# sahaRatul/sela

Hardware: NVIDIA H100
Metric: encode+decode MSamples/s (higher is better)
Workload: dtype f64+int64

## Files before the change

### sela_b200/csrc/c_abi.cu

```cuda
#include <algorithm>
#include <atomic>
#include <cmath>
#include <cstdarg>
#include <cstddef>
#include <cstdio>
#include <cstdlib>
#include <cstring>
#include <mutex>
#include <thread>
#include <vector>

#include "lossless.cuh"
#include "pairing.cuh"
#include "search.cuh"
#include "search_guided.cuh"
#include "search_pairing.cuh"
#include "verify.cuh"
#include "window.cuh"

using namespace selab200;

namespace {

thread_local char g_error[512] = "";
// ... 728 lines not shown
            wp.mask = o.windows;
            wp.n = n_windows;
            wp.su = reinterpret_cast<SearchUnit *>(ws + l.window_search);
            wp.key = reinterpret_cast<unsigned long long *>(ws + l.window_keys);
            wp.n_window = o.d_n_window;
            wp.pred = o.d_window_pred;
            wp.trace = o.d_search_trace;
            const bool trace = o.d_search_trace != nullptr;
            if (int rc = stereo ? launch_windows<true>(p, wp, su, n_frames, n_units, o.d_base_words, stream, trace)
                                : launch_windows<false>(p, wp, su, n_frames, n_units, o.d_base_words, stream, trace))
                return rc;
        }
    } else {
        const int rc_units = stereo ? (o.d_trace ? launch_encode_units<true, true>(p, n_units, o.d_trace, stream)
                                                 : launch_encode_units<true, false>(p, n_units, nullptr, stream))
                                    : (o.d_trace ? launch_encode_units<false, true>(p, n_units, o.d_trace, stream)
                                                 : launch_encode_units<false, false>(p, n_units, nullptr, stream));
        if (rc_units)
            return rc_units;
    }
    const unsigned scan_ctas = (unsigned)((n_sub + kScanTile - 1) / kScanTile);
    k_encode_sizes<<<scan_ctas, kScanTile, 0, stream>>>(p);
    if (int rc = launch_check("k_encode_sizes"))
        return rc;
    if (o.before_scan)
        CUDA_TRY(cudaStreamWaitEvent(stream, o.before_scan, 0));
    k_encode_scan<<<scan_ctas, kScanTile, 0, stream>>>(p);
    if (int rc = launch_check("k_encode_scan"))
        return rc;
    CUDA_TRY(cudaMemcpyAsync(d_used, p.residues, 8, cudaMemcpyDeviceToDevice, stream));
    if (pairing) {
        k_pairing_patch<<<(unsigned)((n_sub + 255) / 256), 256, 0, stream>>>(p, q);
        if (int rc = launch_check("k_pairing_patch"))
            return rc;
    }
    if (o.h_fill_after)
        CUDA_TRY(cudaMemcpyAsync(o.h_fill_after, d_used, 8, cudaMemcpyDeviceToHost, stream));
    if (o.after_scan)
        CUDA_TRY(cudaEventRecord(o.after_scan, stream));
    if (o.d_container) {
        k_encode_gather_container<<<(unsigned)((n_sub + 7) / 8), 256, 0, stream>>>(p, o.d_container, o.sub_base);
        return launch_check("k_encode_gather_container");
    }
    k_encode_gather<<<(unsigned)((n_sub + 7) / 8), 256, 0, stream>>>(p);
    return launch_check("k_encode_gather");
}

int launch_rice_decode(const DecodeParams &p, int which, cudaStream_t stream)
{
    const size_t n_sub = (size_t)p.n_frames * p.channels;
    const unsigned blocks = (unsigned)((n_sub + 32 * kRiceWarps - 1) / (32 * kRiceWarps));
    k_rice_decode<kRiceRing, kRiceBatch><<<blocks, 32 * kRiceWarps, 0, stream>>>(p, which);
    return launch_check(which ? "k_rice_decode(res)" : "k_rice_decode(refl)");
}

int rice_split_log2(size_t n_sub)
{
    if (const char *env = std::getenv("SELAB200_RICE_SPLIT")) {
        const long v = std::atol(env);
        if (v <= 0)
            return -1;
        int l = 0;
        while ((1 << (l + 1)) <= v && l < 4)
            l++;
        return l;
    }
    const size_t sms = (size_t)g.sms;
    if (n_sub >= 81 * sms)
        return 0;
    int l = 0;
    while (l < 4 && (n_sub << l) < 270 * sms)
        l++;
    return l;
}

template <int LOG2S>
int launch_split_index(const RiceVsParams &q, size_t n_sub, cudaStream_t stream)
{
    const unsigned blocks = (unsigned)(((n_sub << LOG2S) + 32 * kVsWarps - 1) / (32 * kVsWarps));
    if (int rc = set_smem(k_rice_split_index<LOG2S>, kSplitSmemBytes))
        return rc;
    k_rice_split_index<LOG2S><<<blocks, 32 * kVsWarps, kSplitSmemBytes, stream>>>(q);
    return launch_check("k_rice_split_index");
}

int launch_rice_residues(const DecodeParams &p, void *aux, cudaStream_t stream)
{
    const size_t n_sub = (size_t)p.n_frames * p.channels;
    const int log2s = rice_split_log2(n_sub);
    if (log2s < 0 || (reinterpret_cast<uintptr_t>(p.ws_res) & 15) != 0) {
        CUDA_TRY(cudaMemsetAsync(static_cast<uint32_t *>(aux) + n_sub * 15, 0, n_sub * 4, stream));
        return launch_rice_decode(p, 1, stream);
    }
    RiceVsParams q;
    q.descs = p.descs;
    q.n_sub = (uint32_t)n_sub;
    q.channels = p.channels;
    q.words = p.words;
    q.n_words = p.n_words;
    q.out = p.ws_res;
    q.table = static_cast<uint32_t *>(aux);
    q.flags = q.table + n_sub * 15;
    q.status = p.status;
    int rc = 0;
    switch (log2s) {
    case 0: CUDA_TRY(cudaMemsetAsync(q.flags, 0, n_sub * 4, stream)); break;
    case 1: rc = launch_split_index<1>(q, n_sub, stream); break;
    case 2: rc = launch_split_index<2>(q, n_sub, stream); break;
    case 3: rc = launch_split_index<3>(q, n_sub, stream); break;
    default: rc = launch_split_index<4>(q, n_sub, stream); break;
    }
    if (rc)
        return rc;
    const size_t n_vs = n_sub << log2s;
    const unsigned vs_blocks = (unsigned)((n_vs + 32 * kVsWarps - 1) / (32 * kVsWarps));
    if (int rc2 = set_smem(k_rice_decode_vc, kVcSmemBytes))
        return rc2;
    k_rice_decode_vc<<<vs_blocks, 32 * kVsWarps, kVcSmemBytes, stream>>>(q, log2s);
    if (int rc2 = launch_check("k_rice_decode_vc"))
        return rc2;
    DecodeParams pf = p;
    pf.rice_flags = q.flags;
    return launch_rice_decode(pf, 1, stream);
}

int decode_device(const selab200_subframe_desc *d_descs, uint32_t n_frames, uint32_t channels,
                  const uint32_t *d_words, size_t n_words, int16_t *d_pcm, int32_t *d_status, void *d_ws,
                  size_t ws_bytes, cudaStream_t stream, bool fresh = true)
{
    if (int rc = check_channels(channels))
        return rc;
    if (ws_bytes < selab200_decode_workspace_bytes(n_frames, channels))
        return fail(SELAB200_ERR_ARGUMENT, "decode workspace too small");
    if (fresh)
        CUDA_TRY(cudaMemsetAsync(d_status, 0, sizeof(int32_t), stream));
    if (n_frames == 0)
        return 0;
    const size_t n_sub = (size_t)n_frames * channels;
    DecodeParams p;
    p.descs = d_descs;
    p.n_frames = n_frames;
    p.channels = channels;
    p.words = d_words;
    p.n_words = n_words;
    p.pcm_out = d_pcm;
    p.status = d_status;
    p.ws_q = static_cast<int32_t *>(d_ws);
    p.ws_res = reinterpret_cast<int32_t *>(static_cast<char *>(d_ws) + align256(n_sub * 128 * 4));
    p.seg_index = reinterpret_cast<uint32_t *>(reinterpret_cast<char *>(p.ws_res) + align256(n_sub * kFrame * 4));
    p.rice_flags = nullptr;
    const size_t n_warps = synthesis_warps(n_sub);
    void *rice_aux = reinterpret_cast<char *>(p.seg_index) + align256(n_warps * 32 * 4);
    CUDA_TRY(cudaMemsetAsync(p.seg_index, 0xff, n_warps * 32 * 4, stream));
    const unsigned plan_ctas = (unsigned)((n_sub + kScanTile - 1) / kScanTile);
    k_decode_width_counts<<<plan_ctas, kScanTile, 0, stream>>>(p, static_cast<WidthCounts *>(rice_aux));
    if (int rc = launch_check("k_decode_width_counts"))
        return rc;
    k_decode_plan<<<plan_ctas, kScanTile, 0, stream>>>(p, static_cast<const WidthCounts *>(rice_aux));
    if (int rc = launch_check("k_decode_plan"))
        return rc;
    if (int rc = launch_rice_decode(p, 0, stream))
        return rc;
    if (int rc = launch_rice_residues(p, rice_aux, stream))
        return rc;
    k_synthesise_segments<<<(unsigned)n_warps, 32, 0, stream>>>(p);
    if (int rc = launch_check("k_synthesise_segments"))
        return rc;
    if (channels == 1)
        return 0;
    k_diff_fixup<<<n_frames, 128, 0, stream>>>(p);
    return launch_check("k_diff_fixup");
}

int read_status(cudaStream_t stream, const int32_t *d_status)
{
    CUDA_TRY(cudaMemcpyAsync(&g.h_small->status, d_status, sizeof(int32_t), cudaMemcpyDeviceToHost, stream));
    CUDA_TRY(cudaStreamSynchronize(stream));
    if (g.h_small->status != 0)
        return fail(g.h_small->status, "%s", status_text(g.h_small->status));
    return 0;
}

int verify_device(const selab200_subframe_desc *d_descs, uint32_t n_frames, uint32_t channels, const uint32_t *d_words,
                  size_t n_words, const int16_t *d_ref, selab200_verify_entry *d_entries, unsigned long long *d_count,
                  int32_t *d_status, void *d_ws, size_t ws_bytes, cudaStream_t stream, bool fresh = true,
                  uint32_t frame_base = 0)
{
    if (int rc = check_channels(channels))
        return rc;
    if (ws_bytes < selab200_verify_workspace_bytes(n_frames, channels))
        return fail(SELAB200_ERR_ARGUMENT, "verify workspace too small");
    if ((reinterpret_cast<uintptr_t>(d_ref) & 15) != 0)
        return fail(SELAB200_ERR_ARGUMENT, "source PCM must be 16-byte aligned on the device");
    const size_t n_sub = (size_t)n_frames * channels;
    if (fresh) {
        CUDA_TRY(cudaMemsetAsync(d_status, 0, sizeof(int32_t), stream));
        CUDA_TRY(cudaMemsetAsync(d_count, 0, sizeof(unsigned long long), stream));
        if (n_sub)
            CUDA_TRY(cudaMemsetAsync(d_entries, 0, n_sub * sizeof(selab200_verify_entry), stream));
    }
    if (n_frames == 0)
        return 0;
    const size_t dec_bytes = align256(selab200_decode_workspace_bytes(n_frames, channels));
    int16_t *d_decoded = reinterpret_cast<int16_t *>(static_cast<char *>(d_ws) + dec_bytes);
    if (int rc = decode_device(d_descs, n_frames, channels, d_words, n_words, d_decoded, d_status, d_ws, dec_bytes,
                               stream, false))
        return rc;
    k_verify_compare<<<n_frames, kVerifyThreads, 0, stream>>>(d_decoded, d_ref, channels, frame_base, d_status,
                                                              d_entries, d_count);
    return launch_check("k_verify_compare");
}

struct VerifyArea {
    unsigned long long *count = nullptr;
    int32_t *status = nullptr;
    selab200_verify_entry *entries = nullptr;
    selab200_subframe_desc *descs = nullptr;
    uint32_t *arena = nullptr;
};

int verify_area(size_t n_sub, size_t arena_words, cudaStream_t stream, VerifyArea &v)
{
    const size_t e_bytes = align256(n_sub * sizeof(selab200_verify_entry));
    const size_t d_bytes = arena_words ? align256(n_sub * sizeof(selab200_subframe_desc)) : 0;
    if (int rc = g.verify.ensure(256 + e_bytes + d_bytes + (arena_words ? arena_words * 4 + 64 : 0)))
        return rc;
    char *b = static_cast<char *>(g.verify.ptr);
    v.count = reinterpret_cast<unsigned long long *>(b);
    v.status = reinterpret_cast<int32_t *>(b + 8);
    v.entries = reinterpret_cast<selab200_verify_entry *>(b + 256);
    v.descs = arena_words ? reinterpret_cast<selab200_subframe_desc *>(b + 256 + e_bytes) : nullptr;
    v.arena = arena_words ? reinterpret_cast<uint32_t *>(b + 256 + e_bytes + d_bytes) : nullptr;
    CUDA_TRY(cudaMemsetAsync(b, 0, 256 + n_sub * sizeof(selab200_verify_entry), stream));
    return 0;
}

bool record_set(const selab200_verify_entry &e) { return e.n_differing != 0; }
bool record_set(const selab200_lossless_entry &e) { return e.words != 0; }

template <typename T>
int collect_records(const unsigned long long *d_count, const int32_t *d_status, const T *d_records, size_t n,
                    cudaStream_t stream, std::vector<T> &out)
{
    out.clear();
    CUDA_TRY(cudaMemcpyAsync(&g.h_small->n_records, d_count, d_status ? 16 : 8, cudaMemcpyDeviceToHost, stream));
    CUDA_TRY(cudaStreamSynchronize(stream));
    const unsigned long long count = g.h_small->n_records;
    const int32_t st = d_status ? g.h_small->records_status : 0;
    if (st != 0)
        return fail(st, "%s", status_text(st));
    if (count == 0)
        return 0;
    std::vector<T> all(n);
    CUDA_TRY(cudaMemcpyAsync(all.data(), d_records, n * sizeof(T), cudaMemcpyDeviceToHost, stream));
    CUDA_TRY(cudaStreamSynchronize(stream));
    out.reserve((size_t)count);
    for (const T &e : all)
        if (record_set(e))
            out.push_back(e);
    return 0;
}

template <typename T>
int deliver_records(const std::vector<T> &records, T *entries, size_t capacity, size_t *n_entries)
{
    *n_entries = records.size();
    if (capacity && !records.empty())
        memcpy(entries, records.data(), std::min(capacity, records.size()) * sizeof(T));
    return 0;
}

}

extern "C" {

int selab200_abi_version(void) { return SELAB200_ABI_VERSION; }
const char *selab200_last_error(void) { return g_error; }
uint64_t selab200_launch_count(void) { return g_launches.load(); }

static int init_slot(int device, int slot)
{
    CUDA_TRY(cudaSetDevice(device));
    cudaDeviceProp prop;
    CUDA_TRY(cudaGetDeviceProperties(&prop, device));
    if (prop.major != 9 || prop.minor != 0)
        return fail(SELAB200_ERR_NO_DEVICE, "device %d is sm_%d%d; this build targets sm_90a only", device,
                    prop.major, prop.minor);
    CUDA_TRY(cudaStreamCreateWithFlags(&g.stream, cudaStreamNonBlocking));
    CUDA_TRY(cudaStreamCreateWithFlags(&g.s_h2d, cudaStreamNonBlocking));
    CUDA_TRY(cudaStreamCreateWithFlags(&g.s_d2h, cudaStreamNonBlocking));
    for (int i = 0; i < kLanes; i++)
        CUDA_TRY(cudaStreamCreateWithFlags(&g.s_compute[i], cudaStreamNonBlocking));
    for (int i = 0; i < kMaxChunks; i++) {
        CUDA_TRY(cudaEventCreateWithFlags(&g.ev_h2d[i], cudaEventDisableTiming));
        CUDA_TRY(cudaEventCreateWithFlags(&g.ev_done[i], cudaEventDisableTiming));
        CUDA_TRY(cudaEventCreateWithFlags(&g.ev_scan[i], cudaEventDisableTiming));
    }
    CUDA_TRY(cudaEventCreateWithFlags(&g.ev_reset, cudaEventDisableTiming));
    g.events = true;
    CUDA_TRY(cudaMallocHost(reinterpret_cast<void **>(&g.h_small), sizeof(Counters)));
    CUDA_TRY(cudaMallocHost(reinterpret_cast<void **>(&g.h_totals), (kMaxChunks + 1) * 8));
    if (int rc = g.small.ensure(256))
        return rc;
    CUDA_TRY(cudaMemcpyToSymbol(d_analysis_windows, analysis_window_table(), sizeof(d_analysis_windows)));
    CUDA_TRY(cudaDeviceSynchronize());
    void *table = nullptr;
    CUDA_TRY(cudaGetSymbolAddress(&table, d_analysis_windows));
    g.windows = static_cast<const double *>(table);
    g.spare = &g_spare_store[slot];
    g.device = device;
    g.sms = prop.multiProcessorCount;
    g.ready = true;
    return 0;
}

static void shutdown_slot()
{
    if (g.device >= 0)
// ... 2095 lines not shown
```

### sela_b200/csrc/kernels.cuh

```cuda
#pragma once

#include "lpc.cuh"
#include "rice.cuh"
#include "rice_vs.cuh"

namespace selab200 {

enum { kMeanPcm = 0, kMeanStereo = 1, kMeanPlanar = 2 };
constexpr int kMeanTile = 64;
constexpr int kMeanSlots = 16;

struct MeanTiling {
    uint32_t units_per_row;
    uint32_t step;
    uint32_t row_stride;
    uint32_t rows_max;
    uint32_t row_words;
};

__host__ __device__ inline MeanTiling mean_tiling(int kind, uint32_t channels)
{
    MeanTiling t;
    uint32_t span = 1;
    if (kind == kMeanPcm) {
// ... 618 lines not shown
    }
    if (lane < (int)(4 - s))
        out[D + lane] = (uint8_t)(src[0] >> (8 * lane));
    else if (lane >= 4 && lane < (int)(4 + s))
        out[D - s + 4ull * n + (lane - 4)] = (uint8_t)(src[n - 1] >> (8 * (4 - s + (lane - 4))));
}

__device__ __forceinline__ void get_words_at_byte(const uint8_t *in, unsigned long long D, uint32_t *dst, uint32_t n)
{
    const int lane = lane_id();
    const uint32_t s = (uint32_t)(D & 3);
    const uint32_t *src = reinterpret_cast<const uint32_t *>(in + (D - s));
    for (uint32_t t0 = lane; t0 < n; t0 += 128) {
        uint32_t v[4];
#pragma unroll
        for (int j = 0; j < 4; j++) {
            const uint32_t t = t0 + 32 * j;
            v[j] = t < n ? (s ? __funnelshift_r(src[t], src[t + 1], 8 * s) : src[t]) : 0u;
        }
#pragma unroll
        for (int j = 0; j < 4; j++)
            if (t0 + 32 * j < n)
                dst[t0 + 32 * j] = v[j];
    }
}

__global__ void __launch_bounds__(256) k_encode_gather_container(EncodeParams p, uint8_t *container,
                                                                 unsigned long long sub_base)
{
    const uint32_t sub = blockIdx.x * 8 + warp_id();
    const uint32_t n_sub = p.n_frames * p.channels;
    if (sub >= n_sub || *reinterpret_cast<volatile int32_t *>(p.status) != 0)
        return;
    const int lane = lane_id();
    const Emit e = choose_unit(p.units, p.channels, sub);
    const selab200_subframe_desc d = p.descs[sub];
    const uint32_t *slot = p.slots + (size_t)e.unit * kSlotWords;
    const unsigned long long g = sub_base + sub;
    const unsigned long long at = container_subframe_byte(g, p.channels, d.refl_offset);
    if (g % p.channels == 0 && lane >= 12 && lane < 16) {
        const uint32_t sync = 0xAA55FF00u;
        container[at - 4 + (lane - 12)] = (uint8_t)(sync >> (8 * (lane - 12)));
    }
    const unsigned long long at2 = at + 7 + 4ull * d.refl_words;
    if (lane < 12) {
        uint8_t v;
        switch (lane) {
        case 0: v = d.channel; break;
        case 1: v = d.subframe_type; break;
        case 2: v = d.parent_channel; break;
        case 3: v = d.refl_rice_param; break;
        case 4: v = (uint8_t)d.refl_words; break;
        case 5: v = (uint8_t)(d.refl_words >> 8); break;
        case 6: v = d.lpc_order; break;
        case 7: v = d.res_rice_param; break;
        case 8: v = (uint8_t)d.res_words; break;
        case 9: v = (uint8_t)(d.res_words >> 8); break;
        case 10: v = (uint8_t)d.samples; break;
        default: v = (uint8_t)(d.samples >> 8); break;
        }
        container[lane < 7 ? at + lane : at2 + (lane - 7)] = v;
    }
    put_words_at_byte(container, at + 7, slot, d.refl_words);
    put_words_at_byte(container, at2 + 5, slot + kSlotReflWords, d.res_words);
}

__global__ void __launch_bounds__(256) k_container_unpack(const uint8_t *container, const selab200_subframe_desc *descs,
                                                          uint32_t n_sub, uint32_t channels, unsigned long long sub_base,
                                                          uint32_t *arena)
{
    const uint32_t sub = blockIdx.x * 8 + warp_id();
    if (sub >= n_sub)
        return;
    const selab200_subframe_desc d = descs[sub];
    const unsigned long long at = container_subframe_byte(sub_base + sub, channels, d.refl_offset);
    get_words_at_byte(container, at + 7, arena + d.refl_offset, d.refl_words);
    get_words_at_byte(container, at + 7 + 4ull * d.refl_words + 5, arena + d.res_offset, d.res_words);
}


__device__ __forceinline__ bool frame_check(const selab200_subframe_desc *fd, uint32_t ch, unsigned long long n_words)
{
    bool ok = true;
    unsigned seen = 0, type_mask = 0;
    for (uint32_t i = 0; i < ch; i++) {
        const selab200_subframe_desc d = fd[i];
        const bool good = desc_ok(d, ch, n_words) && !((seen >> d.channel) & 1);
        ok &= good;
        if (good) {
            seen |= 1u << d.channel;
            type_mask |= (unsigned)(d.subframe_type & 1) << d.channel;
        }
    }
    for (uint32_t i = 0; i < ch && ok; i++) {
        const selab200_subframe_desc d = fd[i];
        if (d.subframe_type == 1 && ((type_mask >> d.parent_channel) & 1))
            ok = false;
    }
    return ok;
}

struct DecodeParams {
    const selab200_subframe_desc *descs;
    uint32_t n_frames, channels;
    const uint32_t *words;
    unsigned long long n_words;
    int16_t *pcm_out;
    int32_t *status;
    int32_t *ws_q;
    int32_t *ws_res;
    uint32_t *seg_index;
    const uint32_t *rice_flags;
};

constexpr int kRiceWarps = 2;
constexpr int kRiceRing = 64, kRiceBatch = 8;
template <int RING, int BATCH>
__global__ void __launch_bounds__(32 * kRiceWarps) k_rice_decode(DecodeParams p, int which)
{
    __shared__ uint32_t ring[kRiceWarps][(RING + 1) * 32];
    const uint32_t sub = blockIdx.x * blockDim.x + threadIdx.x;
    const uint32_t n_sub = p.n_frames * p.channels;
    RiceLaneStream st;
    st.src = p.words;
    st.n_words = 0;
    st.k = 0;
    st.count = 0;
    st.out = nullptr;
    if (sub < n_sub) {
        const selab200_subframe_desc d = p.descs[sub];
        if (!desc_ok(d, p.channels, p.n_words)) {
            raise_status(p.status, SELAB200_ERR_BITSTREAM);
        } else if (which == 0) {
            st.src = p.words + d.refl_offset;
            st.n_words = d.refl_words;
            st.k = d.refl_rice_param;
            st.count = d.lpc_order;
            st.out = p.ws_q + (size_t)sub * 128;
        } else if (!p.rice_flags || p.rice_flags[sub]) {
            st.src = p.words + d.res_offset;
            st.n_words = d.res_words;
            st.k = d.res_rice_param;
            st.count = d.samples;
            st.out = p.ws_res + (size_t)sub * kFrame;
        }
    }
    if (which == 1 && p.rice_flags && __ballot_sync(kFull, st.count != 0) == 0)
        return;
    if (!warp_rice_decode32<RING, BATCH>(ring[warp_id()], st))
        raise_status(p.status, SELAB200_ERR_BITSTREAM);
}

constexpr uint32_t kNoSegment = 0xffffffffu;
constexpr int kMaxTemplates = 2 * kMaxWidth;

struct WidthCounts {
    uint32_t n[16];
};
struct SegTemplate {
    uint32_t repeats, first_warp;
    uint8_t copies[16], lane0[16];
};

__device__ __forceinline__ int subframe_width(const DecodeParams &p, uint32_t u)
{
    const int order = p.descs[u].lpc_order;
    return segment_width(order > kMaxOrder ? 0 : order);
}

__device__ __forceinline__ uint32_t warp_width_counts(int w, uint32_t (*cnt)[16])
{
    const int lane = lane_id();
    uint32_t rank = 0;
#pragma unroll
    for (int v = 0; v < 16; v++) {
        const unsigned b = __ballot_sync(kFull, w == v);
        if (w == v)
            rank = __popc(b & ((1u << lane) - 1u));
        if (lane == 0)
            cnt[warp_id()][v] = __popc(b);
    }
    return rank;
}

__global__ void __launch_bounds__(kScanTile) k_decode_width_counts(DecodeParams p, WidthCounts *tmp)
{
    __shared__ uint32_t cnt[32][16];
    const uint32_t u = blockIdx.x * kScanTile + threadIdx.x;
    warp_width_counts(u < p.n_frames * p.channels ? subframe_width(p, u) : 0, cnt);
    __syncthreads();
    if (threadIdx.x < 16) {
        uint32_t s = 0;
        for (int w = 0; w < 32; w++)
            s += cnt[w][threadIdx.x];
        tmp[blockIdx.x].n[threadIdx.x] = s;
    }
}

__device__ int segment_templates(uint32_t (&c)[16], SegTemplate *tpl)
{
    int nt = 0;
    uint32_t warp = 0;
    for (;;) {
        SegTemplate t;
        int room = 32;
        uint32_t rep = 0xffffffffu;
#pragma unroll
        for (int v = 15; v >= 1; v--) {
            const uint32_t k = v > kMaxWidth ? 0u : min(c[v], (uint32_t)(room / v));
            t.copies[v] = (uint8_t)k;
            t.lane0[v] = (uint8_t)(32 - room);
            room -= (int)k * v;
            if (k)
                rep = min(rep, c[v] / k);
        }
        if (room == 32)
            return nt;
#pragma unroll
        for (int v = 1; v < 16; v++)
            c[v] -= rep * t.copies[v];
        t.copies[0] = t.lane0[0] = 0;
        t.repeats = rep;
        t.first_warp = warp;
        warp += rep;
        tpl[nt++] = t;
    }
}

__global__ void __launch_bounds__(kScanTile) k_decode_plan(DecodeParams p, const WidthCounts *tmp)
{
    __shared__ uint32_t cnt[32][16];
    __shared__ uint32_t part_all[kScanTile / 16][16], part_before[kScanTile / 16][16];
    __shared__ uint32_t total[16], before[16];
    __shared__ SegTemplate tpl[kMaxTemplates];
    const uint32_t n_units = p.n_frames * p.channels;
    const uint32_t u = blockIdx.x * kScanTile + threadIdx.x;
    const int w = u < n_units ? subframe_width(p, u) : 0;
    const uint32_t rank = warp_width_counts(w, cnt);
    {
        const int v = threadIdx.x & 15, g = threadIdx.x >> 4;
        uint32_t all = 0, pre = 0;
        for (uint32_t b = g; b < gridDim.x; b += kScanTile / 16) {
            const uint32_t x = tmp[b].n[v];
            all += x;
            if (b < blockIdx.x)
                pre += x;
        }
        part_all[g][v] = all;
        part_before[g][v] = pre;
    }
    __syncthreads();
    if (threadIdx.x < 16) {
        const int v = threadIdx.x;
        uint32_t all = 0, pre = 0, run = 0;
        for (int g = 0; g < kScanTile / 16; g++)
            all += part_all[g][v], pre += part_before[g][v];
        total[v] = all;
        before[v] = pre;
        for (int x = 0; x < 32; x++) {
            const uint32_t c = cnt[x][v];
            cnt[x][v] = run;
            run += c;
        }
    }
    __syncthreads();
    if (threadIdx.x == 0) {
        uint32_t c[16];
#pragma unroll
        for (int v = 0; v < 16; v++)
            c[v] = v ? total[v] : 0u;
        segment_templates(c, tpl);
    }
    __syncthreads();
    if (u >= n_units)
        return;
    const uint32_t r = before[w] + cnt[warp_id()][w] + rank;
    uint32_t acc = 0;
    int t = 0;
    for (;; t++) {
        const uint32_t m = tpl[t].repeats * tpl[t].copies[w];
        if (r < acc + m)
            break;
        acc += m;
    }
    const uint32_t k = tpl[t].copies[w], j = r - acc, rep = j / k;
    const uint32_t lane = tpl[t].lane0[w] + (j - rep * k) * (uint32_t)w;
    p.seg_index[((size_t)tpl[t].first_warp + rep) * 32 + lane] = u;
}

__host__ __device__ inline size_t synthesis_warps(size_t n_sub) { return n_sub / 2 + 1; }

__global__ void __launch_bounds__(32) k_synthesise_segments(DecodeParams p)
{
    __shared__ __align__(16) SegSmem sm;
    const uint32_t ch = p.channels;
    const int lane = lane_id();
    const uint32_t entry = p.seg_index[(size_t)blockIdx.x * 32 + lane];
    const unsigned starts = __ballot_sync(kFull, entry != kNoSegment);
    if (!(starts & 1u))
        return;
    const int start = 31 - __clz(starts & (0xffffffffu >> (31 - lane)));
    const uint32_t sub = __shfl_sync(kFull, entry, start);
    const int seg = __popc(starts & ((1u << start) - 1u));
    const int n_seg = __popc(starts);
    const int k = lane - start;
    const uint32_t frame = sub / ch, pos = sub % ch;
    const selab200_subframe_desc *fd = p.descs + (size_t)frame * ch;
    const int n = subframe_width(p, sub);
    const bool exists = k < n;

    const bool frame_ok = frame_check(fd, ch, p.n_words);
    if (!frame_ok && k == 0)
        raise_status(p.status, SELAB200_ERR_BITSTREAM);
    const selab200_subframe_desc mine = fd[pos];
    const bool proc = exists && frame_ok;
    const bool diff = proc && mine.subframe_type == 1;
    int16_t *out = p.pcm_out + (size_t)frame * kFrame * ch;
    int32_t *row = p.ws_res + (size_t)sub * kFrame;
    if (k == 0) {
        sm.row_res[seg] = row;
        sm.row_out[seg] = diff ? static_cast<void *>(row) : static_cast<void *>(out + mine.channel);
        sm.row_mode[seg] = !proc ? 0 : diff ? 2 : 1;
    }
    __syncwarp();
    segment_synthesis(sm, start, k, n, seg, n_seg, proc ? mine.lpc_order : 0, p.ws_q + (size_t)sub * 128, ch);

    if (exists && !frame_ok) {
        for (int t = k; t < kFrame; t += n)
            out[(size_t)t * ch + pos] = 0;
    }
}

__global__ void __launch_bounds__(128) k_diff_fixup(DecodeParams p)
{
    const uint32_t frame = blockIdx.x, ch = p.channels;
    const selab200_subframe_desc *fd = p.descs + (size_t)frame * ch;
    bool any = false;
    for (uint32_t pos = 0; pos < ch; pos++)
        any |= fd[pos].subframe_type == 1;
    if (!any || !frame_check(fd, ch, p.n_words))
        return;
    int16_t *out = p.pcm_out + (size_t)frame * kFrame * ch;
    for (uint32_t pos = 0; pos < ch; pos++) {
        const selab200_subframe_desc d = fd[pos];
        if (d.subframe_type != 1)
            continue;
        const int32_t *diff = p.ws_res + ((size_t)frame * ch + pos) * kFrame;
        for (int t = threadIdx.x; t < kFrame; t += blockDim.x)
            out[(size_t)t * ch + d.channel] =
                (int16_t)(uint16_t)((uint32_t)out[(size_t)t * ch + d.parent_channel] - (uint32_t)diff[t]);
    }
}


struct Row17 {
    __align__(16) int16_t a[kHistoryPad + kFrame];
    uint32_t lo[(kHistoryPad + kFrame) / 32];
    __device__ __forceinline__ Signal stage(const int32_t *src)
    {
        const int lane = lane_id();
        for (int i = lane; i < kHistoryPad / 2; i += 32)
            reinterpret_cast<uint32_t *>(a)[i] = 0;
        if (lane < kHistoryPad / 32)
            lo[lane] = 0;
        stage_17bit_row(src, a + kHistoryPad, lo + kHistoryPad / 32);
        __syncwarp();
        return Signal{a + kHistoryPad, lo + kHistoryPad / 32};
    }
};

__global__ void __launch_bounds__(32) k_lpc_residues(const int32_t *samples, const double *means, uint32_t n_sub,
                                                     uint8_t *order_out, int32_t *q_out, int32_t *residues)
{
    __shared__ __align__(16) AnalysisScratch scratch;
    __shared__ __align__(16) CoefSmem cf;
    __shared__ __align__(16) Row17 row;
    const uint32_t sub = blockIdx.x;
    const int lane = lane_id();
    const Signal sig = row.stage(samples + (size_t)sub * kFrame);
    warp_autocorrelation(sig, scratch, means[sub]);
    warp_schur(scratch);
    const int order = warp_order_and_quantise(scratch, cf);
    warp_coefficients(cf, scratch.t(), order);
    warp_fir_residual<true>(sig, cf, order, reinterpret_cast<uint32_t *>(scratch.ring), residues + (size_t)sub * kFrame);
    for (int i = lane; i < kMaxOrder; i += 32)
        q_out[(size_t)sub * kMaxOrder + i] = i < order ? cf.q[i] : 0;
    if (lane == 0)
        order_out[sub] = (uint8_t)order;
}

template <bool CHECK = false>
__global__ void __launch_bounds__(32) k_fir_probe(const int32_t *samples, const int32_t *orders, const long long *c,
                                                  int wide, int32_t *residues, uint8_t *ties)
{
    __shared__ __align__(16) AnalysisScratch scratch;
    __shared__ __align__(16) CoefSmem cf;
    __shared__ __align__(16) Row17 row;
    const uint32_t sub = blockIdx.x;
    const int lane = lane_id();
    const int32_t *src = samples + (size_t)sub * kFrame;
    Signal sig = row.stage(src);
    if (!wide) {
        for (int j = lane; j < kFrame; j += 32)
            row.a[kHistoryPad + j] = (int16_t)src[j];
        sig.lo = nullptr;
    }
    const int order = orders[sub];
    for (int i = lane; i < 112; i += 32) {
        const long long v = i < order ? c[(size_t)sub * (kMaxOrder + 1) + i + 1] : 0;
        cf.clo[i] = (uint32_t)v;
        cf.chi[i] = (int32_t)(v >> 32);
    }
    __syncwarp();
    uint32_t *planes = reinterpret_cast<uint32_t *>(scratch.ring);
    int32_t *res = residues + (size_t)sub * kFrame;
    const bool tie = wide ? warp_fir_residual<true, CHECK>(sig, cf, order, planes, res)
                          : warp_fir_residual<false, CHECK>(sig, cf, order, planes, res);
    if (CHECK && lane == 0)
        ties[sub] = tie;
}

__global__ void __launch_bounds__(32) k_lpc_samples(const int32_t *residues, uint32_t n_sub, const uint8_t *order_in,
                                                    const int32_t *q_in, int32_t *samples)
{
    __shared__ __align__(16) SegSmem sm;
    const uint32_t sub = blockIdx.x;
    const int lane = lane_id();
    const int order = min((int)order_in[sub], kMaxOrder);
    const int n = segment_width(order);
    if (lane == 0) {
        sm.row_res[0] = residues + (size_t)sub * kFrame;
        sm.row_out[0] = samples + (size_t)sub * kFrame;
        sm.row_mode[0] = 2;
    }
    __syncwarp();
    segment_synthesis(sm, 0, lane, n, 0, 1, lane < n ? order : 0, q_in + (size_t)sub * kMaxOrder, 1);
}

__global__ void k_quantise_probe(const double *k, uint32_t n, int32_t *out)
{
    const uint32_t i = blockIdx.x * blockDim.x + threadIdx.x;
    if (i >= n)
        return;
    const double kv = k[i];
    out[4 * (size_t)i + 0] = quantise_reflection(0, kv);
    out[4 * (size_t)i + 1] = quantise_reflection(1, kv);
    out[4 * (size_t)i + 2] = quantise_reflection(2, kv);
    out[4 * (size_t)i + 3] = reflection_significant(kv) ? 1 : 0;
}

__global__ void k_selftest_scaling(uint32_t *mismatches)
{
    const int s = (int)(blockIdx.x * blockDim.x + threadIdx.x) - 65535;
    if (s > 65535)
        return;
    if (__double_as_longlong(sample_to_x(s)) != __double_as_longlong(sample_to_x_div(s)))
        atomicAdd(mismatches, 1u);
}

__global__ void __launch_bounds__(32) k_rice_encode(const int32_t *values, const uint32_t *counts, uint32_t pitch,
                                                    uint32_t *k_out, uint32_t *n_words_out, uint32_t *words,
                                                    uint32_t words_stride, int32_t *status)
{
    const uint32_t st = blockIdx.x;
    const int32_t *v = values + (size_t)st * pitch;
    const int n = (int)counts[st];
    RiceChoice c = warp_rice_choose(v, n);
    if (lane_id() == 0) {
        k_out[st] = c.k;
        n_words_out[st] = c.words;
    }
    if (c.words > words_stride) {
        if (lane_id() == 0)
            raise_status(status, SELAB200_ERR_CAPACITY);
        return;
    }
    warp_rice_pack(v, n, c, words + (size_t)st * words_stride);
}

__global__ void __launch_bounds__(32 * kRiceWarps) k_rice_decode_streams(
    const uint32_t *words, const uint32_t *n_words, uint32_t words_stride, const uint32_t *k,
    const uint32_t *counts, uint32_t n_streams, int32_t *out, uint32_t out_stride, int32_t *status)
{
    __shared__ uint32_t ring[kRiceWarps][(kRiceRing + 1) * 32];
    const uint32_t st_i = blockIdx.x * blockDim.x + threadIdx.x;
    RiceLaneStream st;
    st.src = words;
    st.n_words = 0;
    st.k = 0;
    st.count = 0;
    st.out = nullptr;
    if (st_i < n_streams) {
        if (k[st_i] >= 32 || counts[st_i] > out_stride || n_words[st_i] > words_stride) {
            raise_status(status, SELAB200_ERR_BITSTREAM);
        } else {
            st.src = words + (size_t)st_i * words_stride;
            st.n_words = n_words[st_i];
            st.k = k[st_i];
            st.count = counts[st_i];
            st.out = out + (size_t)st_i * out_stride;
        }
    }
    warp_rice_decode32<kRiceRing, kRiceBatch>(ring[warp_id()], st);
}

}
```

### sela_b200/csrc/lpc.cuh

```cuda
#pragma once

#include "common.cuh"
#include "lpc_tables.cuh"

namespace selab200 {

struct CoefSmem {
    uint32_t clo[112];
    int32_t  chi[112];
    int32_t  q[104];
};
struct AnalysisScratch {
    double ring[256];
    double ac[128];
    __device__ __forceinline__ double *kk() { return ring; }
    __device__ __forceinline__ double *t() { return ring + 104; }
};
using LpcSmem = AnalysisScratch;
constexpr size_t kCoefAlias = 208 * sizeof(double);

__device__ __forceinline__ long long coef_at(const CoefSmem &cf, int j)
{
    return (long long)(((unsigned long long)(uint32_t)cf.chi[j - 1] << 32) | cf.clo[j - 1]);
}
// ... 369 lines not shown
                    sum = mad_wide_s32(T[k][r], 1 << (8 * k), sum);
                const uint32_t top = (uint32_t)T[4][r] + ((uint32_t)T[5][r] << 8) + ((uint32_t)T[6][r] << 16) +
                                     ((uint32_t)T[7][r] << 24);
                sum += (unsigned long long)top << 32;
                out[e] = s[e] - (int32_t)((long long)sum >> kQ);
                if constexpr (CHECK)
                    tie |= (int32_t)((long long)sum >> kQ) + (int32_t)((long long)((1ull << kQ) - sum) >> kQ) != 0;
            }
            *reinterpret_cast<int2 *>(res + i) = make_int2(out[0], out[1]);
        }
    }
    __syncwarp();
    if constexpr (CHECK)
        return __any_sync(kFull, tie);
    return false;
}

constexpr int kTapsPerLane = 8;
constexpr int kMaxWidth = (kMaxOrder + kTapsPerLane - 1) / kTapsPerLane;
constexpr int kSegBlock = 16;
constexpr int kSegRow = 20;
static_assert(kSegBlock % kTapsPerLane == 0, "the register of slot 0 must be static inside a block");

__device__ __forceinline__ int segment_width(int order)
{
    return order <= kTapsPerLane ? 1 : (order + kTapsPerLane - 1) / kTapsPerLane;
}

struct SegSmem {
    int32_t q[32 * kTapsPerLane];
    union {
        double t[32 * kTapsPerLane];
        int32_t out[32 * kSegRow];
    };
    int32_t in[2][32 * kSegRow];
    const int32_t *row_res[32];
    void *row_out[32];
    int row_mode[32];
};

__device__ __forceinline__ void segment_coefficients(SegSmem &sm, int start, int k, int n, int order, int order_max,
                                                     uint32_t (&cl)[kTapsPerLane], uint32_t (&ch)[kTapsPerLane])
{
    double *t = sm.t + kTapsPerLane * start;
    const int32_t *q = sm.q + kTapsPerLane * start;
    const bool live = order > 1 && k < n;
    for (int i = 0; i < order_max; i++) {
        if (live && i < order) {
            const double ki = dequantise(i, q[i]);
            const int half = i >> 1;
            for (int j = k; j < half; j += n) {
                double a = t[j];
                double b = t[i - 1 - j];
                t[j] = dadd(a, dmul(ki, b));
                t[i - 1 - j] = dadd(b, dmul(ki, a));
            }
            if (k == 0) {
                if (i & 1) {
                    double mid = t[half];
                    t[half] = dadd(mid, dmul(mid, ki));
                }
                t[i] = ki;
            }
        }
        __syncwarp();
    }
    const double scale = 34359738368.0;
#pragma unroll
    for (int m = 0; m < kTapsPerLane; m++) {
        const int j = kTapsPerLane * k + m;
        const long long v = (live && j < order) ? __double2ll_rz(dmul(scale, -t[j])) : 0;
        cl[m] = (uint32_t)v;
        ch[m] = (uint32_t)((unsigned long long)v >> 32);
    }
    __syncwarp();
}

struct SegState {
    uint32_t cl[kTapsPerLane];
    uint32_t ch[kTapsPerLane];
    unsigned long long acc[kTapsPerLane];
    uint32_t sp;
    unsigned long long fresh;
};

__device__ __forceinline__ void segment_state(SegState &st, int k, int n, int src)
{
    unsigned long long tot = 0, loc[kTapsPerLane];
#pragma unroll
    for (int m = kTapsPerLane - 1; m >= 0; m--) {
        loc[m] = tot;
        tot += ((unsigned long long)st.ch[m] << 32) | st.cl[m];
    }
    unsigned long long incl = tot;
#pragma unroll
    for (int o = 1; o < 32; o <<= 1) {
        const unsigned long long x = __shfl_down_sync(kFull, incl, o);
        if (k + o < n)
            incl += x;
    }
    const unsigned long long above = incl - tot;
    st.fresh = ~((1ull << (kQ - 1)) + (__shfl_sync(kFull, incl, src) << 31));
#pragma unroll
    for (int m = 0; m < kTapsPerLane; m++)
        st.acc[m] = ((above + loc[m]) << 31) + st.fresh;
}

__device__ __forceinline__ unsigned long long segment_tap(unsigned long long acc, uint32_t cl, uint32_t ch, uint32_t sp)
{
    unsigned long long d;
    asm("{\n\t.reg .u32 lo, hi;\n\t"
        "mov.b64 {lo, hi}, %4;\n\t"
        "mad.lo.u32 hi, %2, %3, hi;\n\t"
        "mad.lo.cc.u32 lo, %1, %3, lo;\n\t"
        "madc.hi.u32 hi, %1, %3, hi;\n\t"
        "mov.b64 %0, {lo, hi};\n\t}"
        : "=l"(d) : "r"(cl), "r"(ch), "r"(sp), "l"(acc));
    return d;
}

template <bool FIRST>
__device__ __forceinline__ void segment_block(SegState &st, const int32_t *in_row, int32_t *out_row, int src, bool top,
                                              bool first)
{
#pragma unroll
    for (int g = 0; g < kSegBlock; g += 4) {
        const int4 r4 = *reinterpret_cast<const int4 *>(in_row + g);
        const uint32_t r[4] = {(uint32_t)r4.x, (uint32_t)r4.y, (uint32_t)r4.z, (uint32_t)r4.w};
        uint32_t s[4];
#pragma unroll
        for (int h = 0; h < 4; h++) {
            const int e = g + h;
            if (FIRST && e == 0) {
                st.sp = r[0] ^ kSynthBias;
            } else {
                const int u = (e + kTapsPerLane - 1) % kTapsPerLane;
#pragma unroll
                for (int m = 0; m < kTapsPerLane; m++)
                    st.acc[(m + u) % kTapsPerLane] =
                        segment_tap(st.acc[(m + u) % kTapsPerLane], st.cl[m], st.ch[m], st.sp);
                const unsigned long long done = st.acc[u];
                const unsigned long long incoming = __shfl_down_sync(kFull, done, 1);
                const uint32_t v = r[h] + (uint32_t)((int32_t)(done >> 32) >> (kQ - 32)) + (1u + kSynthBias);
                st.sp = __shfl_sync(kFull, v, src);
                st.acc[u] = top ? st.fresh : incoming;
            }
            s[h] = st.sp;
        }
        if (first)
            *reinterpret_cast<int4 *>(out_row + g) = make_int4((int)s[0], (int)s[1], (int)s[2], (int)s[3]);
    }
}

__device__ __forceinline__ void segment_synthesis(SegSmem &sm, int start, int k, int n, int seg, int n_seg, int order,
                                                  const int32_t *q, uint32_t stride)
{
    const int lane = lane_id();
    auto fetch = [&](int B) {
        for (int i = lane >> 2; i < n_seg; i += 8) {
            const int32_t *src = sm.row_res[i] + kSegBlock * B + 4 * (lane & 3);
            const uint32_t dst = (uint32_t)__cvta_generic_to_shared(&sm.in[B & 1][i * kSegRow + 4 * (lane & 3)]);
            asm volatile("cp.async.cg.shared.global [%0], [%1], 16;" ::"r"(dst), "l"(src) : "memory");
        }
        asm volatile("cp.async.commit_group;" ::: "memory");
    };
    fetch(0);
    fetch(1);

    for (int i = k; i < order; i += n)
        sm.q[kTapsPerLane * start + i] = q[i];
    __syncwarp();
    int order_max = order;
#pragma unroll
    for (int o = 16; o; o >>= 1)
        order_max = max(order_max, __shfl_xor_sync(kFull, order_max, o));
    SegState st;
    segment_coefficients(sm, start, k, n, order, order_max, st.cl, st.ch);
    segment_state(st, k, n, start);

    const bool top = k == n - 1, first = k == 0;
    int32_t *out_row = sm.out + seg * kSegRow;
    for (int B = 0; B < kFrame / kSegBlock; B++) {
        asm volatile("cp.async.wait_group 1;" ::: "memory");
        __syncwarp();
        const int32_t *in_row = sm.in[B & 1] + seg * kSegRow;
        if (B == 0)
            segment_block<true>(st, in_row, out_row, start, top, first);
        else
            segment_block<false>(st, in_row, out_row, start, top, first);
        __syncwarp();
        for (int i = lane >> 4; i < n_seg; i += 2) {
            const int mode = sm.row_mode[i];
            const int e = lane & 15, t = kSegBlock * B + e;
            const int v = (int)((uint32_t)sm.out[i * kSegRow + e] ^ kSynthBias);
            if (mode == 1)
                static_cast<int16_t *>(sm.row_out[i])[(size_t)t * stride] = (int16_t)(uint16_t)v;
            else if (mode == 2)
                static_cast<int32_t *>(sm.row_out[i])[t] = v;
        }
        if (B + 2 < kFrame / kSegBlock)
            fetch(B + 2);
        else
            asm volatile("cp.async.commit_group;" ::: "memory");
    }
}

}
```

Before: 12890.

## Plan decode segments per frame and fuse stereo fixup into interleaved synthesis output

For mono or stereo output with 16-byte aligned PCM, the decode plan now packs whole frames, so all of a frame's channels go into one synthesis warp. Synthesis then writes interleaved int16 PCM with vectorized stores and applies the difference-channel reconstruction inline, which removes the separate k_diff_fixup launch and its scattered strided 16-bit writes. The width-count and template planning is also rewritten to be warp-parallel, using match_any and per-lane templates instead of a single-thread loop. The trade-offs are more complex row_mode encoding and wider plan arrays, and packing may be less dense when frame widths are large.

```diff
diff --git a/sela_b200/csrc/c_abi.cu b/sela_b200/csrc/c_abi.cu
--- a/sela_b200/csrc/c_abi.cu
+++ b/sela_b200/csrc/c_abi.cu
@@ -904,18 +904,27 @@
     const size_t n_warps = synthesis_warps(n_sub);
     void *rice_aux = reinterpret_cast<char *>(p.seg_index) + align256(n_warps * 32 * 4);
     CUDA_TRY(cudaMemsetAsync(p.seg_index, 0xff, n_warps * 32 * 4, stream));
-    const unsigned plan_ctas = (unsigned)((n_sub + kScanTile - 1) / kScanTile);
-    k_decode_width_counts<<<plan_ctas, kScanTile, 0, stream>>>(p, static_cast<WidthCounts *>(rice_aux));
+    const bool frames = channels <= 2 && reinterpret_cast<uintptr_t>(d_pcm) % 16 == 0;
+    const size_t n_units = frames ? n_frames : n_sub;
+    const unsigned plan_ctas = (unsigned)((n_units + kScanTile - 1) / kScanTile);
+    k_decode_width_counts<<<plan_ctas, kScanTile, 0, stream>>>(p, static_cast<WidthCounts *>(rice_aux), frames);
     if (int rc = launch_check("k_decode_width_counts"))
         return rc;
-    k_decode_plan<<<plan_ctas, kScanTile, 0, stream>>>(p, static_cast<const WidthCounts *>(rice_aux));
+    k_decode_plan<<<plan_ctas, kScanTile, 0, stream>>>(p, static_cast<const WidthCounts *>(rice_aux), frames);
     if (int rc = launch_check("k_decode_plan"))
         return rc;
     if (int rc = launch_rice_decode(p, 0, stream))
         return rc;
     if (int rc = launch_rice_residues(p, rice_aux, stream))
         return rc;
-    k_synthesise_segments<<<(unsigned)n_warps, 32, 0, stream>>>(p);
+    if (frames) {
+        if (channels == 1)
+            k_synthesise_segments<1><<<(unsigned)n_warps, 32, 0, stream>>>(p);
+        else
+            k_synthesise_segments<2><<<(unsigned)n_warps, 32, 0, stream>>>(p);
+        return launch_check("k_synthesise_segments");
+    }
+    k_synthesise_segments<0><<<(unsigned)n_warps, 32, 0, stream>>>(p);
     if (int rc = launch_check("k_synthesise_segments"))
         return rc;
     if (channels == 1)
diff --git a/sela_b200/csrc/kernels.cuh b/sela_b200/csrc/kernels.cuh
--- a/sela_b200/csrc/kernels.cuh
+++ b/sela_b200/csrc/kernels.cuh
@@ -794,14 +794,15 @@
 }
 
 constexpr uint32_t kNoSegment = 0xffffffffu;
-constexpr int kMaxTemplates = 2 * kMaxWidth;
+constexpr int kPlanWidths = 32;
+constexpr int kMaxTemplates = 2 * 2 * kMaxWidth;
 
 struct WidthCounts {
-    uint32_t n[16];
+    uint32_t n[kPlanWidths];
 };
 struct SegTemplate {
     uint32_t repeats, first_warp;
-    uint8_t copies[16], lane0[16];
+    uint8_t copies[kPlanWidths], lane0[kPlanWidths];
 };
 
 __device__ __forceinline__ int subframe_width(const DecodeParams &p, uint32_t u)
@@ -810,28 +811,40 @@
     return segment_width(order > kMaxOrder ? 0 : order);
 }
 
-__device__ __forceinline__ uint32_t warp_width_counts(int w, uint32_t (*cnt)[16])
-{
-    const int lane = lane_id();
-    uint32_t rank = 0;
-#pragma unroll
-    for (int v = 0; v < 16; v++) {
-        const unsigned b = __ballot_sync(kFull, w == v);
-        if (w == v)
-            rank = __popc(b & ((1u << lane) - 1u));
-        if (lane == 0)
-            cnt[warp_id()][v] = __popc(b);
-    }
-    return rank;
-}
-
-__global__ void __launch_bounds__(kScanTile) k_decode_width_counts(DecodeParams p, WidthCounts *tmp)
-{
-    __shared__ uint32_t cnt[32][16];
+__device__ __forceinline__ int unit_width(const DecodeParams &p, uint32_t u, bool frames)
+{
+    if (!frames)
+        return subframe_width(p, u);
+    int w = 0;
+    for (uint32_t c = 0; c < p.channels; c++)
+        w += subframe_width(p, u * p.channels + c);
+    return w;
+}
+
+__device__ __forceinline__ uint32_t warp_width_counts(int w, uint32_t (*cnt)[kPlanWidths])
+{
+    static_assert(kPlanWidths == 32, "a lane per width");
+    const int lane = lane_id();
+    const unsigned same = __match_any_sync(kFull, w);
+    cnt[warp_id()][lane] = 0;
+    __syncwarp();
+    if (lane == __ffs(same) - 1)
+        cnt[warp_id()][w] = __popc(same);
+    return __popc(same & ((1u << lane) - 1u));
+}
+
+__device__ __forceinline__ uint32_t plan_units(const DecodeParams &p, bool frames)
+{
+    return frames ? p.n_frames : p.n_frames * p.channels;
+}
+
+__global__ void __launch_bounds__(kScanTile) k_decode_width_counts(DecodeParams p, WidthCounts *tmp, bool frames)
+{
+    __shared__ uint32_t cnt[32][kPlanWidths];
     const uint32_t u = blockIdx.x * kScanTile + threadIdx.x;
-    warp_width_counts(u < p.n_frames * p.channels ? subframe_width(p, u) : 0, cnt);
+    warp_width_counts(u < plan_units(p, frames) ? unit_width(p, u, frames) : 0, cnt);
     __syncthreads();
-    if (threadIdx.x < 16) {
+    if (threadIdx.x < kPlanWidths) {
         uint32_t s = 0;
         for (int w = 0; w < 32; w++)
             s += cnt[w][threadIdx.x];
@@ -839,50 +852,57 @@
     }
 }
 
-__device__ int segment_templates(uint32_t (&c)[16], SegTemplate *tpl)
-{
-    int nt = 0;
+__device__ int segment_templates(uint32_t c, SegTemplate *tpl)
+{
+    const int lane = lane_id();
     uint32_t warp = 0;
-    for (;;) {
-        SegTemplate t;
+    for (int nt = 0;; nt++) {
+        const unsigned live = __ballot_sync(kFull, c != 0);
+        if (!live)
+            return nt;
         int room = 32;
-        uint32_t rep = 0xffffffffu;
-#pragma unroll
-        for (int v = 15; v >= 1; v--) {
-            const uint32_t k = v > kMaxWidth ? 0u : min(c[v], (uint32_t)(room / v));
-            t.copies[v] = (uint8_t)k;
-            t.lane0[v] = (uint8_t)(32 - room);
-            room -= (int)k * v;
-            if (k)
-                rep = min(rep, c[v] / k);
-        }
-        if (room == 32)
-            return nt;
-#pragma unroll
-        for (int v = 1; v < 16; v++)
-            c[v] -= rep * t.copies[v];
-        t.copies[0] = t.lane0[0] = 0;
-        t.repeats = rep;
-        t.first_warp = warp;
+        uint32_t k = 0, l0 = 0;
+        for (unsigned m = live;;) {
+            m &= room >= 31 ? ~0u : (2u << room) - 1u;
+            if (!m)
+                break;
+            const int v = 31 - __clz(m);
+            m ^= 1u << v;
+            const uint32_t kv = min(__shfl_sync(kFull, c, v), (uint32_t)room / (uint32_t)v);
+            if (lane == v) {
+                k = kv;
+                l0 = 32 - room;
+            }
+            room -= (int)kv * v;
+        }
+        const uint32_t rep = __reduce_min_sync(kFull, k ? c / k : 0xffffffffu);
+        c -= rep * k;
+        SegTemplate &t = tpl[nt];
+        t.copies[lane] = (uint8_t)k;
+        t.lane0[lane] = (uint8_t)l0;
+        if (lane == 0) {
+            t.repeats = rep;
+            t.first_warp = warp;
+        }
         warp += rep;
-        tpl[nt++] = t;
-    }
-}
-
-__global__ void __launch_bounds__(kScanTile) k_decode_plan(DecodeParams p, const WidthCounts *tmp)
-{
-    __shared__ uint32_t cnt[32][16];
-    __shared__ uint32_t part_all[kScanTile / 16][16], part_before[kScanTile / 16][16];
-    __shared__ uint32_t total[16], before[16];
+    }
+}
+
+__global__ void __launch_bounds__(kScanTile) k_decode_plan(DecodeParams p, const WidthCounts *tmp, bool frames)
+{
+    constexpr int kGroups = kScanTile / kPlanWidths;
+    __shared__ uint32_t cnt[32][kPlanWidths];
+    __shared__ uint32_t part_all[kGroups][kPlanWidths], part_before[kGroups][kPlanWidths];
+    __shared__ uint32_t total[kPlanWidths], before[kPlanWidths];
     __shared__ SegTemplate tpl[kMaxTemplates];
-    const uint32_t n_units = p.n_frames * p.channels;
+    const uint32_t n_units = plan_units(p, frames);
     const uint32_t u = blockIdx.x * kScanTile + threadIdx.x;
-    const int w = u < n_units ? subframe_width(p, u) : 0;
+    const int w = u < n_units ? unit_width(p, u, frames) : 0;
     const uint32_t rank = warp_width_counts(w, cnt);
     {
-        const int v = threadIdx.x & 15, g = threadIdx.x >> 4;
+        const int v = threadIdx.x % kPlanWidths, g = threadIdx.x / kPlanWidths;
         uint32_t all = 0, pre = 0;
-        for (uint32_t b = g; b < gridDim.x; b += kScanTile / 16) {
+        for (uint32_t b = g; b < gridDim.x; b += kGroups) {
             const uint32_t x = tmp[b].n[v];
             all += x;
             if (b < blockIdx.x)
@@ -892,10 +912,10 @@
         part_before[g][v] = pre;
     }
     __syncthreads();
-    if (threadIdx.x < 16) {
+    if (threadIdx.x < kPlanWidths) {
         const int v = threadIdx.x;
         uint32_t all = 0, pre = 0, run = 0;
-        for (int g = 0; g < kScanTile / 16; g++)
+        for (int g = 0; g < kGroups; g++)
             all += part_all[g][v], pre += part_before[g][v];
         total[v] = all;
         before[v] = pre;
@@ -906,13 +926,8 @@
         }
     }
     __syncthreads();
-    if (threadIdx.x == 0) {
-        uint32_t c[16];
-#pragma unroll
-        for (int v = 0; v < 16; v++)
-            c[v] = v ? total[v] : 0u;
-        segment_templates(c, tpl);
-    }
+    if (threadIdx.x < 32)
+        segment_templates(threadIdx.x ? total[threadIdx.x] : 0u, tpl);
     __syncthreads();
     if (u >= n_units)
         return;
@@ -926,16 +941,26 @@
         acc += m;
     }
     const uint32_t k = tpl[t].copies[w], j = r - acc, rep = j / k;
-    const uint32_t lane = tpl[t].lane0[w] + (j - rep * k) * (uint32_t)w;
-    p.seg_index[((size_t)tpl[t].first_warp + rep) * 32 + lane] = u;
+    uint32_t lane = tpl[t].lane0[w] + (j - rep * k) * (uint32_t)w;
+    uint32_t *warp = p.seg_index + ((size_t)tpl[t].first_warp + rep) * 32;
+    if (!frames) {
+        warp[lane] = u;
+        return;
+    }
+    for (uint32_t c = 0; c < p.channels; c++) {
+        const uint32_t sub = u * p.channels + c;
+        warp[lane] = sub;
+        lane += subframe_width(p, sub);
+    }
 }
 
 __host__ __device__ inline size_t synthesis_warps(size_t n_sub) { return n_sub / 2 + 1; }
 
+template <int CH>
 __global__ void __launch_bounds__(32) k_synthesise_segments(DecodeParams p)
 {
     __shared__ __align__(16) SegSmem sm;
-    const uint32_t ch = p.channels;
+    const uint32_t ch = CH ? CH : p.channels;
     const int lane = lane_id();
     const uint32_t entry = p.seg_index[(size_t)blockIdx.x * 32 + lane];
     const unsigned starts = __ballot_sync(kFull, entry != kNoSegment);
@@ -961,15 +986,27 @@
     int32_t *row = p.ws_res + (size_t)sub * kFrame;
     if (k == 0) {
         sm.row_res[seg] = row;
-        sm.row_out[seg] = diff ? static_cast<void *>(row) : static_cast<void *>(out + mine.channel);
-        sm.row_mode[seg] = !proc ? 0 : diff ? 2 : 1;
+        if constexpr (CH == 0) {
+            sm.row_out[seg] = diff ? static_cast<void *>(row) : static_cast<void *>(out + mine.channel);
+            sm.row_mode[seg] = !proc ? 0 : diff ? 2 : 1;
+        } else {
+            if (pos == 0)
+                sm.row_out[seg / CH] = out;
+            const int a = diff ? seg ^ 1 : seg, sub_from = diff || !frame_ok;
+            sm.row_mode[seg - pos + (frame_ok ? mine.channel : pos)] = a | seg << 8 | sub_from << 16;
+        }
     }
     __syncwarp();
-    segment_synthesis(sm, start, k, n, seg, n_seg, proc ? mine.lpc_order : 0, p.ws_q + (size_t)sub * 128, ch);
-
-    if (exists && !frame_ok) {
-        for (int t = k; t < kFrame; t += n)
-            out[(size_t)t * ch + pos] = 0;
+    const int order = proc ? mine.lpc_order : 0;
+    const int32_t *q = p.ws_q + (size_t)sub * 128;
+    if constexpr (CH == 0) {
+        segment_synthesis(sm, start, k, n, seg, n_seg, order, q, [&](int B) { segment_rows_out(sm, B, n_seg, ch); });
+        if (exists && !frame_ok) {
+            for (int t = k; t < kFrame; t += n)
+                out[(size_t)t * ch + pos] = 0;
+        }
+    } else {
+        segment_synthesis(sm, start, k, n, seg, n_seg, order, q, [&](int B) { segment_frames_out<CH>(sm, B, n_seg / CH); });
     }
 }
 
@@ -1076,7 +1113,8 @@
         sm.row_mode[0] = 2;
     }
     __syncwarp();
-    segment_synthesis(sm, 0, lane, n, 0, 1, lane < n ? order : 0, q_in + (size_t)sub * kMaxOrder, 1);
+    segment_synthesis(sm, 0, lane, n, 0, 1, lane < n ? order : 0, q_in + (size_t)sub * kMaxOrder,
+                      [&](int B) { segment_rows_out(sm, B, 1, 1); });
 }
 
 __global__ void k_quantise_probe(const double *k, uint32_t n, int32_t *out)
diff --git a/sela_b200/csrc/lpc.cuh b/sela_b200/csrc/lpc.cuh
--- a/sela_b200/csrc/lpc.cuh
+++ b/sela_b200/csrc/lpc.cuh
@@ -545,8 +545,56 @@
     }
 }
 
+__device__ __forceinline__ void segment_rows_out(const SegSmem &sm, int B, int n_seg, uint32_t stride)
+{
+    const int lane = lane_id();
+    for (int i = lane >> 4; i < n_seg; i += 2) {
+        const int mode = sm.row_mode[i];
+        const int e = lane & 15, t = kSegBlock * B + e;
+        const int v = (int)((uint32_t)sm.out[i * kSegRow + e] ^ kSynthBias);
+        if (mode == 1)
+            static_cast<int16_t *>(sm.row_out[i])[(size_t)t * stride] = (int16_t)(uint16_t)v;
+        else if (mode == 2)
+            static_cast<int32_t *>(sm.row_out[i])[t] = v;
+    }
+}
+
+template <int CH>
+__device__ __forceinline__ void segment_frames_out(const SegSmem &sm, int B, int n_frames)
+{
+    static_assert(CH == 1 || CH == 2, "a frame of more channels does not fit a warp");
+    constexpr int kLanes = 2 * CH, kSpan = kSegBlock / kLanes;
+    const int lane = lane_id();
+    const int e0 = kSpan * (lane % kLanes);
+    for (int f = lane / kLanes; f < n_frames; f += 32 / kLanes) {
+        uint32_t v[CH][kSpan];
+#pragma unroll
+        for (int c = 0; c < CH; c++) {
+            const uint32_t src = (uint32_t)sm.row_mode[CH * f + c];
+            const int32_t *a = sm.out + (src & 0xffu) * kSegRow + e0;
+            const int32_t *b = sm.out + ((src >> 8) & 0xffu) * kSegRow + e0;
+            const uint32_t m = src >> 16 ? ~0u : 0u;
+#pragma unroll
+            for (int j = 0; j < kSpan; j += 4) {
+                const int4 x = *reinterpret_cast<const int4 *>(a + j), y = *reinterpret_cast<const int4 *>(b + j);
+                v[c][j + 0] = (uint32_t)x.x - ((uint32_t)y.x & m);
+                v[c][j + 1] = (uint32_t)x.y - ((uint32_t)y.y & m);
+                v[c][j + 2] = (uint32_t)x.z - ((uint32_t)y.z & m);
+                v[c][j + 3] = (uint32_t)x.w - ((uint32_t)y.w & m);
+            }
+        }
+        uint32_t w[4];
+#pragma unroll
+        for (int i = 0; i < 4; i++)
+            w[i] = prmt(v[(2 * i) % CH][(2 * i) / CH], v[(2 * i + 1) % CH][(2 * i + 1) / CH], 0x5410);
+        int16_t *out = static_cast<int16_t *>(sm.row_out[f]) + (size_t)(kSegBlock * B + e0) * CH;
+        *reinterpret_cast<int4 *>(out) = make_int4((int)w[0], (int)w[1], (int)w[2], (int)w[3]);
+    }
+}
+
+template <typename CopyOut>
 __device__ __forceinline__ void segment_synthesis(SegSmem &sm, int start, int k, int n, int seg, int n_seg, int order,
-                                                  const int32_t *q, uint32_t stride)
+                                                  const int32_t *q, CopyOut copy_out)
 {
     const int lane = lane_id();
     auto fetch = [&](int B) {
@@ -582,15 +630,7 @@
         else
             segment_block<false>(st, in_row, out_row, start, top, first);
         __syncwarp();
-        for (int i = lane >> 4; i < n_seg; i += 2) {
-            const int mode = sm.row_mode[i];
-            const int e = lane & 15, t = kSegBlock * B + e;
-            const int v = (int)((uint32_t)sm.out[i * kSegRow + e] ^ kSynthBias);
-            if (mode == 1)
-                static_cast<int16_t *>(sm.row_out[i])[(size_t)t * stride] = (int16_t)(uint16_t)v;
-            else if (mode == 2)
-                static_cast<int32_t *>(sm.row_out[i])[t] = v;
-        }
+        copy_out(B);
         if (B + 2 < kFrame / kSegBlock)
             fetch(B + 2);
         else
```

After: 13080 (median of 6 runs). 1.02x the previous value.
